# thrill/thrill

Measured on AMD Instinct MI355X. Metric: TeraSort keys/sec (100-byte recs), higher is better.
Workload: dtype u8; 1 GPU; terasort_10GiB_100B; records=107374182, record_bytes=100, seed=0x7421, parallelism=dp1

## Files before the change

thrill_amd/csrc/t9_rank_scatter.h:

```cpp
#pragma once
#include "t9_common.h"

template <int NDIG>
__device__ inline void t9_scan_onewave(u32* s_vals, u32 tid) {
    if (tid < 64) {
        const u32 lane = tid;
        u32 carry = 0;
        for (int c = 0; c < NDIG / 64; ++c) {
            const u32 v0 = s_vals[c * 64 + lane];
            u32 v = v0;
            for (int off = 1; off < 64; off <<= 1) {
                u32 y = __shfl_up(v, off);
                if (lane >= (u32)off) v += y;
            }
            const u32 total = __shfl(v, 63);
            s_vals[c * 64 + lane] = (v - v0) + carry;
            carry += total;
        }
    }
}

__device__ inline void t9_scan256_onewave(u32* s_vals, u32 tid) {
    if (tid < 64) {
        const u32 lane = tid;
        u32 carry = 0;
        for (int c = 0; c < 4; ++c) {
            const u32 v0 = s_vals[c * 64 + lane];
            u32 v = v0;
            for (int off = 1; off < 64; off <<= 1) {
                u32 y = __shfl_up(v, off);
                if (lane >= (u32)off) v += y;
            }
            const u32 total = __shfl(v, 63);
            s_vals[c * 64 + lane] = (v - v0) + carry;
            carry += total;
        }
    }
}

template <int BITS>
__device__ inline void t9_hist_ballot_add(u32* __restrict__ s_cnt, u32 d,
                                          bool valid, u32 lane) {
    u64 m = __ballot(valid);
    for (int b = 0; b < BITS; ++b) {
        const u64 bb = __ballot((d >> b) & 1u);
        m &= ((d >> b) & 1u) ? bb : ~bb;
    }
    if (valid && (u32)__popcll(m & ((1ull << lane) - 1ull)) == 0)
        atomicAdd(&s_cnt[d], (u32)__popcll(m));
}

template <int TILE, int BLOCK, bool HAS_KEY, bool HAS_VAL,
          int REC_WORDS = 0, bool IOTA_VAL = false>
__global__ __launch_bounds__(BLOCK, 8) void k_scatter_wave512(
    const u64* __restrict__ in_keys, const u32* __restrict__ in_vals,
    u64* __restrict__ out_keys, u32* __restrict__ out_vals,
    const u32* __restrict__ offs, u64 n, u32 shift) {
    constexpr int NW = BLOCK / 64;
    constexpr int SUB = TILE / NW;
    constexpr int GROUPS = SUB / 64;
    static_assert(HAS_KEY, "the store phase reads the digit from the key");
    static_assert(TILE % BLOCK == 0 && SUB % 64 == 0, "whole groups");
    const u32* rec32 = (const u32*)in_keys;
    __shared__ __align__(16) u8 s_raw[TILE * 8];
    u64* const s_okeys = (u64*)s_raw;
    u32* const s_ovals = (u32*)s_raw;
    static_assert(TILE <= 65535, "u16 counts and offsets");
    __shared__ u16 s_wcnt[NW * T9_RADIX];
    __shared__ u32 s_start[T9_RADIX];
    __shared__ u32 s_goff[T9_RADIX];

    const u32 tid = threadIdx.x, wave = tid >> 6, lane = tid & 63;
    const u64 base = (u64)blockIdx.x * TILE;
    const u32 tn = (u32)((n - base < (u64)TILE) ? (n - base) : (u64)TILE);

    if (tid < T9_RADIX)
        s_goff[tid] = offs[(u64)blockIdx.x * T9_RADIX + tid];
    u16* const wc = s_wcnt + wave * T9_RADIX;
    for (u32 t = lane; t < T9_RADIX; t += 64) wc[t] = 0;

    u32 pos[GROUPS];
    const u32 wbase = wave * SUB;
#pragma unroll
    for (int g = 0; g < GROUPS; ++g) {
        const u32 i = wbase + g * 64 + lane;
        const bool valid = i < tn;
        u32 d = 0;
        if (valid) {
            if (REC_WORDS)
                d = ((const u8*)rec32)[(base + i) * (u64)REC_WORDS * 4 +
                                       (7 - shift / 8)];
            else
                d = (u32)(in_keys[base + i] >> shift) & 255u;
        }
        u64 m = __ballot(valid);
        for (int bit = 0; bit < 8; ++bit) {
            u64 bb = __ballot((d >> bit) & 1u);
            m &= ((d >> bit) & 1u) ? bb : ~bb;
        }
        const u32 wr = (u32)__popcll(m & ((1ull << lane) - 1ull));
        const u32 before = valid ? (u32)wc[d] : 0;
        pos[g] = before + wr;
        if (valid && wr == 0) wc[d] = (u16)(before + (u32)__popcll(m));
    }
    __syncthreads();

    if (tid < T9_RADIX) {
        u32 run = 0;
        for (int w = 0; w < NW; ++w) {
            const u32 c = s_wcnt[w * T9_RADIX + tid];
            s_wcnt[w * T9_RADIX + tid] = (u16)run;
            run += c;
        }
        s_start[tid] = run;
    }
    __syncthreads();
    t9_scan256_onewave(s_start, tid);
    __syncthreads();

    constexpr bool LOAD_VAL = HAS_VAL && !REC_WORDS && !IOTA_VAL;
    u32 val[LOAD_VAL ? GROUPS : 1];
#pragma unroll
    for (int g = 0; g < GROUPS; ++g) {
        const u32 i = wbase + g * 64 + lane;
        if (i < tn) {
            u64 k;
            if (REC_WORDS) {
                const u64 w0 = (u64)rec32[(base + i) * REC_WORDS];
                const u64 w1 = (u64)rec32[(base + i) * REC_WORDS + 1];
                k = ((u64)__builtin_bswap32((u32)w0) << 32) |
                    __builtin_bswap32((u32)w1);
            }
            else {
                k = in_keys[base + i];
            }
            if constexpr (LOAD_VAL) val[g] = in_vals[base + i];
            const u32 d = (u32)(k >> shift) & 255u;
            pos[g] += s_start[d] + (u32)wc[d];
            s_okeys[pos[g]] = k;
        }
    }
    __syncthreads();

    u32 gpos[GROUPS];
#pragma unroll
    for (int c = 0; c < GROUPS; ++c) {
        const u32 j = c * BLOCK + tid;
        if (j < tn) {
            const u64 k = s_okeys[j];
            const u32 d = (u32)(k >> shift) & 255u;
            gpos[c] = s_goff[d] + (j - s_start[d]);
            out_keys[gpos[c]] = k;
        }
    }
    if (!HAS_VAL) return;
    __syncthreads();

#pragma unroll
    for (int g = 0; g < GROUPS; ++g) {
        const u32 i = wbase + g * 64 + lane;
        if (i < tn) {
            if constexpr (LOAD_VAL) s_ovals[pos[g]] = val[g];
            else s_ovals[pos[g]] = (u32)(base + i);
        }
    }
    __syncthreads();
#pragma unroll
    for (int c = 0; c < GROUPS; ++c) {
        const u32 j = c * BLOCK + tid;
        if (j < tn) out_vals[gpos[c]] = s_ovals[j];
    }
}
```

Measured before the change: 10.67 billion keys/s.

## Load keys once into registers, pack positions, and remap tiles per XCD

```diff
diff --git a/thrill_amd/csrc/t9_rank_scatter.h b/thrill_amd/csrc/t9_rank_scatter.h
--- a/thrill_amd/csrc/t9_rank_scatter.h
+++ b/thrill_amd/csrc/t9_rank_scatter.h
@@ -61,6 +61,7 @@
     constexpr int GROUPS = SUB / 64;
     static_assert(HAS_KEY, "the store phase reads the digit from the key");
     static_assert(TILE % BLOCK == 0 && SUB % 64 == 0, "whole groups");
+    static_assert(GROUPS % 2 == 0, "positions are kept two to a register");
     const u32* rec32 = (const u32*)in_keys;
     __shared__ __align__(16) u8 s_raw[TILE * 8];
     u64* const s_okeys = (u64*)s_raw;
@@ -71,22 +72,48 @@
     __shared__ u32 s_goff[T9_RADIX];
 
     const u32 tid = threadIdx.x, wave = tid >> 6, lane = tid & 63;
-    const u64 base = (u64)blockIdx.x * TILE;
+    const u32 xper = gridDim.x >> 3, xrem = gridDim.x & 7;
+    const u32 xcd = blockIdx.x & 7;
+    const u32 tile = xcd * xper + (xcd < xrem ? xcd : xrem) +
+                     (blockIdx.x >> 3);
+    const u64 base = (u64)tile * TILE;
     const u32 tn = (u32)((n - base < (u64)TILE) ? (n - base) : (u64)TILE);
 
+    constexpr bool ONE_READ = !REC_WORDS;
+    constexpr bool LOAD_VAL = HAS_VAL && !REC_WORDS && !IOTA_VAL;
+    const u32 wbase = wave * SUB;
+    u64 key[ONE_READ ? GROUPS : 1];
+    u32 val[LOAD_VAL ? GROUPS : 1];
+    if constexpr (ONE_READ) {
+#pragma unroll
+        for (int g = 0; g < GROUPS; ++g) {
+            const u32 i = wbase + g * 64 + lane;
+            key[g] = in_keys[base + (i < tn ? i : tn - 1)];
+        }
+        if constexpr (LOAD_VAL) {
+#pragma unroll
+            for (int g = 0; g < GROUPS; ++g) {
+                const u32 i = wbase + g * 64 + lane;
+                val[g] = in_vals[base + (i < tn ? i : tn - 1)];
+            }
+        }
+    }
+
     if (tid < T9_RADIX)
-        s_goff[tid] = offs[(u64)blockIdx.x * T9_RADIX + tid];
+        s_goff[tid] = offs[(u64)tile * T9_RADIX + tid];
     u16* const wc = s_wcnt + wave * T9_RADIX;
     for (u32 t = lane; t < T9_RADIX; t += 64) wc[t] = 0;
 
-    u32 pos[GROUPS];
-    const u32 wbase = wave * SUB;
+    u32 pos2[GROUPS / 2] = {};
 #pragma unroll
     for (int g = 0; g < GROUPS; ++g) {
         const u32 i = wbase + g * 64 + lane;
         const bool valid = i < tn;
         u32 d = 0;
-        if (valid) {
+        if constexpr (ONE_READ) {
+            d = (u32)(key[g] >> shift) & 255u;
+        }
+        else if (valid) {
             if (REC_WORDS)
                 d = ((const u8*)rec32)[(base + i) * (u64)REC_WORDS * 4 +
                                        (7 - shift / 8)];
@@ -100,8 +127,14 @@
         }
         const u32 wr = (u32)__popcll(m & ((1ull << lane) - 1ull));
         const u32 before = valid ? (u32)wc[d] : 0;
-        pos[g] = before + wr;
+        pos2[g >> 1] |= (before + wr) << (16 * (g & 1));
         if (valid && wr == 0) wc[d] = (u16)(before + (u32)__popcll(m));
+    }
+    if constexpr (ONE_READ) {
+#pragma unroll
+        for (int g = 0; g < GROUPS; ++g) asm volatile("" : "+v"(key[g]));
+#pragma unroll
+        for (int q = 0; q < GROUPS / 2; ++q) asm volatile("" : "+v"(pos2[q]));
     }
     __syncthreads();
 
@@ -118,14 +151,15 @@
     t9_scan256_onewave(s_start, tid);
     __syncthreads();
 
-    constexpr bool LOAD_VAL = HAS_VAL && !REC_WORDS && !IOTA_VAL;
-    u32 val[LOAD_VAL ? GROUPS : 1];
 #pragma unroll
     for (int g = 0; g < GROUPS; ++g) {
         const u32 i = wbase + g * 64 + lane;
         if (i < tn) {
             u64 k;
-            if (REC_WORDS) {
+            if constexpr (ONE_READ) {
+                k = key[g];
+            }
+            else if (REC_WORDS) {
                 const u64 w0 = (u64)rec32[(base + i) * REC_WORDS];
                 const u64 w1 = (u64)rec32[(base + i) * REC_WORDS + 1];
                 k = ((u64)__builtin_bswap32((u32)w0) << 32) |
@@ -134,10 +168,12 @@
             else {
                 k = in_keys[base + i];
             }
-            if constexpr (LOAD_VAL) val[g] = in_vals[base + i];
+            if constexpr (LOAD_VAL && !ONE_READ) val[g] = in_vals[base + i];
             const u32 d = (u32)(k >> shift) & 255u;
-            pos[g] += s_start[d] + (u32)wc[d];
-            s_okeys[pos[g]] = k;
+            const u32 add = s_start[d] + (u32)wc[d];
+            const u32 pos = ((pos2[g >> 1] >> (16 * (g & 1))) & 0xffffu) + add;
+            s_okeys[pos] = k;
+            pos2[g >> 1] += add << (16 * (g & 1));
         }
     }
     __syncthreads();
@@ -160,8 +196,9 @@
     for (int g = 0; g < GROUPS; ++g) {
         const u32 i = wbase + g * 64 + lane;
         if (i < tn) {
-            if constexpr (LOAD_VAL) s_ovals[pos[g]] = val[g];
-            else s_ovals[pos[g]] = (u32)(base + i);
+            const u32 pos = (pos2[g >> 1] >> (16 * (g & 1))) & 0xffffu;
+            if constexpr (LOAD_VAL) s_ovals[pos] = val[g];
+            else s_ovals[pos] = (u32)(base + i);
         }
     }
     __syncthreads();
```

After: 10.95 billion keys/s (median of 6 runs). 1.03x the previous value.
